# marksgraham/ddpm-ood

Hardware: AMD Instinct MI355X
Metric: reconstructions/sec (whole node), FashionMNIST 32x32 (higher is better)
Workload: dtype f32 (split-f16 MFMA products, fp32 accumulate)

## Files before the change

### ddpm_ood_amd/_lib.py

```python

from __future__ import annotations

import ctypes as C
import os
from pathlib import Path

import torch

_LIB = None
LIB_NAME = "libddpm_ood_hip.so"
ABI_VERSION = 10


class HipLibraryMissing(RuntimeError):
    pass


class ConvDesc(C.Structure):
    _fields_ = [
        ("in1", C.c_void_p), ("in2", C.c_void_p), ("C1", C.c_int), ("C2", C.c_int),
        ("w_packed", C.c_void_p), ("w_raw", C.c_void_p), ("bias", C.c_void_p),
        ("gscale", C.c_void_p), ("gshift", C.c_void_p),
        ("chan_add", C.c_void_p), ("chan_add_stride", C.c_int),
        ("residual", C.c_void_p), ("out", C.c_void_p),
        ("B", C.c_int), ("Cout", C.c_int),
        ("Hi", C.c_int), ("Wi", C.c_int), ("Ho", C.c_int), ("Wo", C.c_int),
        ("ksize", C.c_int), ("mode", C.c_int), ("act", C.c_int), ("force_direct", C.c_int),
        ("Di", C.c_int), ("Do", C.c_int), ("dims", C.c_int), ("depth_taps", C.c_int),
        ("w_folded", C.c_void_p), ("out_act", C.c_int), ("reserved", C.c_int), ("w_wino", C.c_void_p),
        ("scratch", C.c_void_p), ("scratch_floats", C.c_size_t), ("w_wino44", C.c_void_p),
        ("w_wino44h", C.c_void_p), ("stats_out", C.c_void_p), ("w_d3h", C.c_void_p),
    ]


MAX_LEVELS = 8


class UNetConfig(C.Structure):
    _fields_ = [
        ("spatial_dims", C.c_int), ("in_channels", C.c_int), ("out_channels", C.c_int),
        ("num_levels", C.c_int),
        ("num_channels", C.c_int * MAX_LEVELS), ("attention_levels", C.c_int * MAX_LEVELS),
        ("num_res_blocks", C.c_int * MAX_LEVELS), ("num_head_channels", C.c_int * MAX_LEVELS),
        ("norm_num_groups", C.c_int), ("norm_eps", C.c_float), ("use_proj_attn", C.c_int),
    ]


class GemmDesc(C.Structure):
    _fields_ = [
        ("A", C.c_void_p), ("B", C.c_void_p), ("C", C.c_void_p),
        ("M", C.c_int), ("N", C.c_int), ("K", C.c_int), ("k_inner", C.c_int),
        ("a_m", C.c_int64), ("a_k", C.c_int64), ("a_k_outer", C.c_int64),
        ("b_n", C.c_int64), ("b_k", C.c_int64), ("b_k_outer", C.c_int64),
        ("c_m", C.c_int64), ("c_n", C.c_int64),
        ("batch", C.c_int), ("batch_inner", C.c_int),
        ("a_batch", C.c_int64), ("a_batch_outer", C.c_int64), ("b_batch", C.c_int64), ("b_batch_outer", C.c_int64),
        ("c_batch", C.c_int64), ("c_batch_outer", C.c_int64),
        ("alpha", C.c_float), ("beta", C.c_float),
        ("scratch", C.c_void_p), ("scratch_floats", C.c_size_t),
        ("split_f16", C.c_int), ("reserved0", C.c_int),
    ]


SIGNATURES = {
    "ddpm_abi_version": (C.c_int, []),
    "ddpm_last_error": (C.c_char_p, []),
    "ddpm_conv_f32": (C.c_int, [C.POINTER(ConvDesc), C.c_void_p]),
    "ddpm_conv_scratch_floats": (C.c_size_t, [C.POINTER(ConvDesc)]),
    "ddpm_conv_takes_wino44h": (C.c_int, [C.POINTER(ConvDesc)]),
    "ddpm_conv_stats_parts": (C.c_int, [C.POINTER(ConvDesc)]),
    "ddpm_conv_kernel_name": (C.c_char_p, [C.POINTER(ConvDesc)]),
    "ddpm_conv_kernel_scratch_floats": (C.c_size_t, [C.POINTER(ConvDesc)]),
    "ddpm_conv_s2h_weight_halves": (C.c_size_t, [C.c_int, C.c_int]),
    "ddpm_pack_conv_s2h_weight": (C.c_int, [C.c_void_p, C.c_void_p, C.c_int, C.c_int, C.c_void_p]),
    "ddpm_conv_d3h_weight_halves": (C.c_size_t, [C.c_int, C.c_int]),
    "ddpm_pack_conv_d3h_weight": (C.c_int, [C.c_void_p, C.c_void_p, C.c_int, C.c_int, C.c_void_p]),
    "ddpm_conv_d1s_weight_halves": (C.c_size_t, [C.c_int, C.c_int]),
    "ddpm_pack_conv_d1s_weight": (C.c_int, [C.c_void_p, C.c_void_p, C.c_int, C.c_int, C.c_int, C.c_int, C.c_void_p]),
    "ddpm_conv1x1_h_weight_halves": (C.c_size_t, [C.c_int, C.c_int]),
    "ddpm_pack_conv1x1_h_weight": (C.c_int, [C.c_void_p, C.c_void_p, C.c_int, C.c_int, C.c_void_p]),
    "ddpm_packed_conv_weight_floats": (C.c_size_t, [C.c_int, C.c_int, C.c_int]),
    "ddpm_pack_conv_weight_f32": (C.c_int, [C.c_void_p, C.c_void_p, C.c_int, C.c_int, C.c_int, C.c_int, C.c_int,
                                            C.c_void_p]),
    "ddpm_pack_conv_weight_taps_f32": (C.c_int, [C.c_void_p, C.c_void_p, C.c_int, C.c_int, C.c_int, C.c_int, C.c_int,
                                                 C.c_void_p]),
    "ddpm_pack_conv3d_weight_f32": (C.c_int, [C.c_void_p, C.c_void_p, C.c_int, C.c_int, C.c_int, C.c_void_p]),
    "ddpm_packed_convtr_weight_floats": (C.c_size_t, [C.c_int, C.c_int, C.c_int]),
    "ddpm_pack_convtr_weight_f32": (C.c_int, [C.c_void_p, C.c_void_p, C.c_int, C.c_int, C.c_int, C.c_void_p]),
    "ddpm_conv3d_k4s2_cin1_f32": (C.c_int, [C.c_void_p] * 4 + [C.c_int] * 6 + [C.c_void_p]),
    "ddpm_convtr3d_parity_weights_f32": (C.c_int, [C.c_void_p, C.c_void_p, C.c_int, C.c_int, C.c_void_p]),
    "ddpm_parity_interleave3_f32": (C.c_int, [C.c_void_p, C.c_void_p, C.c_int64, C.c_int, C.c_int, C.c_int, C.c_void_p]),
    "ddpm_convtr3d_k4s2_cout1_f32": (C.c_int, [C.c_void_p] * 4 + [C.c_int] * 5 + [C.c_void_p]),
    "ddpm_wino_weight_floats": (C.c_size_t, [C.c_int, C.c_int]),
    "ddpm_pack_wino_weight_f32": (C.c_int, [C.c_void_p, C.c_void_p, C.c_int, C.c_int, C.c_void_p]),
    "ddpm_wino44_weight_floats": (C.c_size_t, [C.c_int, C.c_int]),
    "ddpm_pack_wino44_weight_f32": (C.c_int, [C.c_void_p, C.c_void_p, C.c_int, C.c_int, C.c_void_p]),
    "ddpm_pack_wino3d_weight_f32": (C.c_int, [C.c_void_p, C.c_void_p, C.c_int, C.c_int, C.c_void_p]),
    "ddpm_convnd_generic_f32": (C.c_int, [C.c_void_p] * 5 + [C.c_int] * 12 + [C.c_void_p]),
    "ddpm_wino44h_weight_halves": (C.c_size_t, [C.c_int, C.c_int]),
    "ddpm_pack_wino44h_weight": (C.c_int, [C.c_void_p, C.c_void_p, C.c_int, C.c_int, C.c_void_p]),
    "ddpm_pack_wino44h_weight3d": (C.c_int, [C.c_void_p, C.c_void_p, C.c_int, C.c_int, C.c_void_p]),
    "ddpm_pack_wino44_weight3d_f32": (C.c_int, [C.c_void_p, C.c_void_p, C.c_int, C.c_int, C.c_void_p]),
    "ddpm_folded_upsample_weight_floats": (C.c_size_t, [C.c_int, C.c_int]),
    "ddpm_fold_upsample_weight_f32": (C.c_int, [C.c_void_p, C.c_void_p, C.c_int, C.c_int, C.c_void_p]),
    "ddpm_gn_scale_shift_f32": (C.c_int, [C.c_void_p, C.c_void_p, C.c_int, C.c_int, C.c_void_p, C.c_void_p,
                                          C.c_void_p, C.c_void_p, C.c_int, C.c_int, C.c_int, C.c_float, C.c_void_p]),
    "ddpm_gn_finalize_f32": (C.c_int, [C.c_void_p, C.c_int, C.c_int, C.c_void_p, C.c_int, C.c_int, C.c_void_p, C.c_void_p,
                                       C.c_void_p, C.c_void_p, C.c_int, C.c_int, C.c_int, C.c_float, C.c_void_p]),
    "ddpm_channel_stats_f32": (C.c_int, [C.c_void_p, C.c_void_p, C.c_int, C.c_int, C.c_int, C.c_void_p]),
    "ddpm_attention_f32": (C.c_int, [C.c_void_p, C.c_void_p, C.c_void_p, C.c_int, C.c_int, C.c_int, C.c_int,
                                     C.c_float, C.c_void_p]),
    "ddpm_attention_scratch_floats": (C.c_size_t, [C.c_int, C.c_int, C.c_int, C.c_int]),
    "ddpm_attention_ws_f32": (C.c_int, [C.c_void_p, C.c_void_p, C.c_void_p, C.c_int, C.c_int, C.c_int, C.c_int,
                                        C.c_float, C.c_void_p, C.c_size_t, C.c_void_p]),
    "ddpm_timestep_embedding_f32": (C.c_int, [C.c_void_p, C.c_void_p, C.c_void_p, C.c_int, C.c_int, C.c_void_p]),
    "ddpm_add_noise_f32": (C.c_int, [C.c_void_p, C.c_void_p, C.POINTER(C.c_float), C.POINTER(C.c_float), C.c_float,
                                     C.c_void_p, C.c_int, C.c_int64, C.c_void_p]),
    "ddpm_plms_step_f32": (C.c_int, [C.c_void_p, C.c_void_p, C.c_void_p, C.c_void_p, C.c_void_p, C.c_int, C.c_int,
                                     C.c_float, C.c_float, C.c_float, C.c_float, C.c_float, C.c_void_p, C.c_int64,
                                     C.c_void_p]),
    "ddpm_ancestral_step_f32": (C.c_int, [C.c_void_p] * 4 + [C.c_int, C.c_int64, C.c_int, C.c_int] + [C.c_float] * 5
                                + [C.c_uint64, C.c_void_p, C.c_void_p]),
    "ddpm_randn_rows_f32": (C.c_int, [C.c_void_p, C.c_int, C.c_int64, C.c_uint64, C.c_void_p, C.c_void_p]),
    "ddpm_vlb_noise_rows_f32": (C.c_int, [C.c_void_p] * 5 + [C.c_int, C.c_void_p, C.c_int, C.c_int64, C.c_void_p]),
    "ddpm_vlb_term_rows_f32": (C.c_int, [C.c_void_p] * 6 + [C.c_int, C.c_int, C.c_int, C.c_float, C.c_void_p, C.c_void_p,
                                         C.c_int, C.c_int64, C.c_void_p]),
    "ddpm_clamp_mse_f32": (C.c_int, [C.c_void_p, C.c_void_p, C.c_float, C.c_void_p, C.c_int, C.c_int64, C.c_void_p]),
    "ddpm_vq_nearest_f32": (C.c_int, [C.c_void_p] * 5 + [C.c_int, C.c_int, C.c_int64, C.c_int, C.c_void_p]),
    "ddpm_vq_train_partials": (C.c_size_t, [C.c_int, C.c_int, C.c_int64]),
    "ddpm_vq_train_assign_f32": (C.c_int, [C.c_void_p] * 9 + [C.c_int, C.c_int, C.c_int64, C.c_int, C.c_float, C.c_void_p]),
    "ddpm_vq_train_update_f32": (C.c_int, [C.c_void_p] * 5 + [C.c_int, C.c_int, C.c_float, C.c_float, C.c_void_p]),
    "ddpm_vq_train_backward_f32": (C.c_int, [C.c_void_p] * 6 + [C.c_int, C.c_int, C.c_int64, C.c_float, C.c_void_p]),
    "ddpm_lpips_conv_f32": (C.c_int, [C.c_void_p] * 6 + [C.c_int] * 10 + [C.c_void_p]),
    "ddpm_maxpool3s2_f32": (C.c_int, [C.c_void_p, C.c_void_p, C.c_int64, C.c_int, C.c_int, C.c_void_p]),
    "ddpm_lpips_conv_biasmap_f32": (C.c_int, [C.c_void_p] * 4 + [C.c_int] * 9 + [C.c_void_p]),
    "ddpm_lpips_conv_mfma_supported": (C.c_int, [C.c_int] * 5),
    "ddpm_lpips_pack_conv_weight_f32": (C.c_int, [C.c_void_p, C.c_void_p, C.c_int, C.c_int, C.c_int, C.c_void_p]),
    "ddpm_lpips_conv_mfma_f32": (C.c_int, [C.c_void_p] * 4 + [C.c_int] * 7 + [C.c_void_p]),
    "ddpm_lpips_layer_f32": (C.c_int, [C.c_void_p] * 4 + [C.c_int] * 4 + [C.c_void_p]),
    "ddpm_sqerr_map_f32": (C.c_int, [C.c_void_p] * 3 + [C.c_int, C.c_int, C.c_int64, C.c_float, C.c_int, C.c_void_p]),
    "ddpm_lpips_layer_map_f32": (C.c_int, [C.c_void_p] * 4 + [C.c_int] * 3 + [C.c_int64, C.c_int64, C.c_void_p]),
    "ddpm_lpips_map_upsample_f32": (C.c_int, [C.c_void_p, C.c_void_p, C.c_int, C.c_int64] + [C.c_int] * 17
                                    + [C.c_float, C.c_int, C.c_void_p]),
    "ddpm_map_stats_update_f32": (C.c_int, [C.c_void_p, C.c_int, C.c_int64, C.c_int64, C.c_void_p, C.c_void_p, C.c_void_p]),
    "ddpm_map_zscore_f32": (C.c_int, [C.c_void_p] * 4 + [C.c_int, C.c_int, C.c_int64, C.c_float, C.c_void_p]),
    "ddpm_map_zscore_loo_f32": (C.c_int, [C.c_void_p] * 5 + [C.c_int, C.c_int, C.c_int64, C.c_int64, C.c_float, C.c_void_p]),
    "ddpm_map_blur_f32": (C.c_int, [C.c_void_p] * 3 + [C.c_int] * 4 + [C.c_void_p]),
    "ddpm_map_blur3d_f32": (C.c_int, [C.c_void_p] * 4 + [C.c_int] * 5 + [C.c_void_p]),
    "ddpm_lpips_map_upsample_view_f32": (C.c_int, [C.c_void_p, C.c_void_p, C.c_int, C.c_int64] + [C.c_int] * 15
                                         + [C.c_float, C.c_int, C.c_void_p]),
    "ddpm_map_mask_hist_f32": (C.c_int, [C.c_void_p, C.c_void_p, C.c_int, C.c_int64, C.c_float, C.c_float, C.c_int, C.c_int,
                                         C.c_void_p, C.c_void_p, C.c_int, C.c_void_p]),
    "ddpm_map_mask_counts_f32": (C.c_int, [C.c_void_p, C.c_void_p, C.c_int, C.c_int64, C.c_void_p, C.c_int, C.c_void_p, C.c_void_p]),
    "ddpm_map_label_u8": (C.c_int, [C.c_void_p, C.c_int, C.c_int, C.c_int, C.c_int, C.c_void_p, C.c_void_p, C.c_void_p]),
    "ddpm_map_label_f32": (C.c_int, [C.c_void_p, C.c_float, C.c_int, C.c_int, C.c_int, C.c_int, C.c_void_p, C.c_void_p, C.c_void_p]),
# ... 182 lines not shown
```

### ddpm_ood_amd/csrc/conv_wino44h.hip

```cpp
#include "wino44h_common.h"

namespace ddpm {

static int w44h_cus() {
  static int cus = 0;
  if (!cus) {
    int dev = 0;
    hipDeviceProp_t prop;
    if (hipGetDevice(&dev) == hipSuccess && hipGetDeviceProperties(&prop, dev) == hipSuccess)
      cus = prop.multiProcessorCount;
    if (cus <= 0) cus = 256;
  }
  return cus;
}

bool w44h_geom(const ddpm_conv_desc &d, W44HGeom &g, bool sizing) {
  const int Cin = d.C1 + d.C2;
  const bool is3d = d.dims == 3;
  const bool up = d.mode == DDPM_CONV_UPSAMPLE2;
  if (d.ksize != 3 || (!is3d && (d.Di > 1 || d.Do > 1)) || (d.mode != DDPM_CONV_NORMAL && !up)) return false;
  if (up) {
    if (!sw().up_wino44h || is3d || d.gscale || d.act != DDPM_ACT_NONE || d.C2 || d.chan_add || d.residual || d.out_act != DDPM_ACT_NONE)
      return false;
    if (d.Ho != 2 * d.Hi || d.Wo != 2 * d.Wi || d.Wo > 32) return false;
  }
  if ((d.out_act != DDPM_ACT_NONE && !(is3d && d.out_act == DDPM_ACT_RELU)) || d.act == DDPM_ACT_RELU) return false;
  if (d.gscale && d.act != DDPM_ACT_SILU) return false;
  if (is3d && (d.gscale || d.act != DDPM_ACT_NONE || d.C2 || d.chan_add)) return false;
  const int Dd = is3d ? (d.Di > 1 ? d.Di : 1) : 1;
  if (is3d && (d.Do > 1 ? d.Do : 1) != Dd) return false;
  if (Cin % 16 || (d.C2 > 0 && d.C1 % 4) || d.Cout % kK) return false;
  if ((d.Ho & 3) || (d.Wo & 3) || (!up && (d.Hi != d.Ho || d.Wi != d.Wo))) return false;
  if ((reinterpret_cast<uintptr_t>(d.out) | reinterpret_cast<uintptr_t>(d.residual)) & 15) return false;
  if ((double)d.B * (d.C1 > d.C2 ? d.C1 : d.C2) * Dd * d.Ho * d.Wo * 4 >= 2147483648.0) return false;
  if ((double)d.B * d.Cout * Dd * d.Ho * d.Wo * 4 >= 2147483648.0 * 2) return false;
  g.TWc = d.Wo / 4;
  g.THr = d.Ho / 4;
  const int per_img = g.TWc * g.THr;
  if (per_img >= kT) {
    if (kT % g.TWc) return false;
    g.TI = 1;
    g.TR = kT / g.TWc;
    if (g.THr % g.TR) return false;
    g.parts = g.THr / g.TR;
  } else {
    if (kT % per_img) return false;
    g.TI = kT / per_img;
    g.TR = g.THr;
    g.parts = 1;
  }
  if (is3d && g.TI != 1) return false;
  g.Cin = Cin;
  g.D = Dd;
  g.NIMG = d.B * Dd;
  g.NCHc = Cin / kC;
  g.kd0 = is3d && Dd == 1 ? 1 : 0;
  g.nkd = is3d && Dd > 1 ? 3 : 1;
  if (is3d && Dd > 1 && (d.depth_taps == 3 || d.depth_taps == 6)) {
    g.kd0 = d.depth_taps == 6 ? 1 : 0;
    g.nkd = 2;
  }
  g.nkd_w = is3d ? 3 : 1;
  g.NCH = g.nkd * g.NCHc;
  g.HW = d.Ho * d.Wo;
  g.up = up;
  g.HWin = up ? d.Hi * d.Wi : g.HW;
  g.CS = Dd * g.HW;
  g.prow = 4 * g.TR + 2;
  w44r_relayout(d, g);
  if (w44h_lds_bytes(g) > 160 * 1024) return false;
  if (64 % d.Wo) return false;
  const int rows = g.prow < d.Ho ? g.prow : d.Ho;
  g.UI = (rows * d.Wo + 63) / 64;
  g.NRT = g.TI * g.UI;
  if (g.TI == 1) {
    if (g.NRT != 9 && g.NRT != 10) return false;
    if ((rows - 1) * d.Wo < 64 * (g.NRT - 1)) return false;
  } else if (!((g.UI == 4 && rows * d.Wo == 256 && g.TI == 2) || (g.UI == 1 && rows * d.Wo == 64 && g.TI == 8))) {
    return false;
  }
  g.KT = d.Cout / kK;
  g.NIT = (g.NIMG + g.TI - 1) / g.TI;
  const long items = (long)g.KT * g.parts * g.NIT;
  const int cus = w44h_cus();
  const bool any_size = sw().conv_wino44 == 2;
  g.S = 1;
  g.pstride = 0;
  if (items < cus && !any_size) {
    if (is3d) return false;
    const int sp_max = sw().wino44_split;
    for (int sp = 4; sp >= 2; sp >>= 1)
      if (sp <= sp_max && items * sp <= cus && g.NCH % (2 * sp) == 0) { g.S = sp; break; }
    if (g.S == 1 || items * g.S * 4 < (long)cus * 3) return false;
    const size_t out_floats = (size_t)d.B * d.Cout * g.HW;
    if (!sizing && (!d.scratch || d.scratch_floats < g.S * out_floats)) return false;
    g.pstride = (long long)out_floats;
  }
  g.IPW = (int)((items + cus - 1) / cus);
  g.NS = g.parts * ((g.NIT + g.IPW - 1) / g.IPW) * g.S;
  while (g.S == 1 && items > cus && (long)g.KT * 8 <= cus && (long)g.KT * ((g.NS + 7) / 8) * 8 > cus && g.IPW < g.NIT) {
    ++g.IPW;
    g.NS = g.parts * ((g.NIT + g.IPW - 1) / g.IPW);
  }
  g.grid = g.KT * ((g.NS + 7) / 8) * 8;
  g.xitem = sw().w44h_xitem;
  g.rev = 0;
  g.xmap = (sw().wino44_xmap >= 0 ? sw().wino44_xmap != 0 : 0) && (8 % g.KT == 0);
  if (g.xmap) g.grid = 8 * ((g.NS + 8 / g.KT - 1) / (8 / g.KT));
  return true;
}

static bool w44h_enabled() {
  return sw().conv_wino44 != 0 && split_f16_on(sw().wino44_f16x3);
}

int conv_wino44h_stats_parts(const ddpm_conv_desc &d) {
  W44HGeom g;
  if (!w44h_enabled() || !d.w_wino44h || d.force_direct || d.dims == 3 || !w44h_geom(d, g, true)) return 0;
  const int per = g.TR * g.TWc;
  if (g.S != 1) return wino_split_reduce_stats_parts(g.HW);
  if ((per != 4 && per != 16 && per != 32) || g.parts > 8) return 0;
  return g.parts;
}

bool conv_wino44h_supported(const ddpm_conv_desc &d) {
  W44HGeom g;
  return w44h_enabled() && d.w_wino44h != nullptr && !d.force_direct && w44h_geom(d, g);
}

size_t conv_wino44h_scratch_floats(const ddpm_conv_desc &d) {
  W44HGeom g;
  if (!w44h_enabled() || !d.w_wino44h || d.force_direct || !w44h_geom(d, g, true) || g.S == 1) return 0;
  return (size_t)g.S * d.B * d.Cout * g.HW;
}

int launch_conv_wino44h(const ddpm_conv_desc &d, hipStream_t s) {
  W44HGeom g;
  if (!d.w_wino44h || !w44h_geom(d, g)) {
    set_error("conv_wino44h: unsupported shape");
    return DDPM_EINVAL;
  }
  ddpm_conv_desc dk = d;
  if (g.S > 1 || conv_wino44h_stats_parts(d) == 0) dk.stats_out = nullptr;
  if (g.S > 1) {
    dk.out = d.scratch;
    dk.bias = nullptr;
    dk.chan_add = nullptr;
    dk.residual = nullptr;
  }
  const double M = (double)g.NIMG * g.HW;
  const double flops = 2.0 * M * d.Cout * (double)g.Cin * 9 * g.nkd;
  const double bytes = 4.0 * ((g.up ? 0.25 : 1.0) * M * g.Cin + M * d.Cout * (d.residual ? 2 : 1) + (double)d.Cout * g.Cin * 9 * g.nkd);
  const char *kname = d.dims == 3 ? "conv3d_wino44h" : g.up ? "conv3x3_wino44h_up" : d.gscale ? "conv3x3_wino44h_gn_silu" : "conv3x3_wino44h";
  char kshape[160];
  if (g_prof_on && sw().prof_shapes) {
    snprintf(kshape, sizeof(kshape), "%s|%d+%d->%d@%dx%d", kname, d.C1, d.C2, d.Cout, d.Ho, d.Wo);
    kname = kshape;
  }
  ProfScope prof(s, kname, flops, bytes);
  static unsigned launch_parity = 0;
  g.rev = sw().w44r_serp ? (int)(launch_parity++ & 1) : 0;
  if (const int rc = launch_conv_wino44r(dk, g, w44h_lds_bytes(g), s)) return rc;
  if (g.S > 1) return launch_wino_split_reduce(d, g.S, g.pstride, g.HW, s);
  return 0;
}

__device__ __forceinline__ void wino44h_u(const float *w, double (&u)[6][6]) {
  const double G[6][3] = {{0.25, 0, 0},           {-1.0 / 6, -1.0 / 6, -1.0 / 6}, {-1.0 / 6, 1.0 / 6, -1.0 / 6},
                          {1.0 / 24, 1.0 / 12, 1.0 / 6}, {1.0 / 24, -1.0 / 12, 1.0 / 6},   {0, 0, 1}};
  double t[6][3];
  for (int r = 0; r < 6; ++r)
    for (int q = 0; q < 3; ++q) t[r][q] = G[r][0] * w[0 * 3 + q] + G[r][1] * w[1 * 3 + q] + G[r][2] * w[2 * 3 + q];
  for (int r = 0; r < 6; ++r)
    for (int c = 0; c < 6; ++c) u[r][c] = t[r][0] * G[c][0] + t[r][1] * G[c][1] + t[r][2] * G[c][2];
}

__global__ void wino44h_max_kernel(const float *__restrict__ src, unsigned *__restrict__ tail, int64_t total) {
  float m = 0.f;
  for (int64_t i = blockIdx.x * (int64_t)blockDim.x + threadIdx.x; i < total; i += (int64_t)gridDim.x * blockDim.x) {
    double u[6][6];
    wino44h_u(src + i * 9, u);
    for (int r = 0; r < 6; ++r)
      for (int c = 0; c < 6; ++c) m = fmaxf(m, fabsf((float)u[r][c]));
  }
  m = wave_max(m);
  if ((threadIdx.x & 63) == 0) atomicMax(tail, __float_as_uint(m));
}

__global__ void wino44h_pack_kernel(const float *__restrict__ src, uint16_t *__restrict__ dst, int Cout, int Cin, int nkd) {
  const int64_t total = (int64_t)Cout * Cin * nkd;
  const int nch = Cin / kC;
  float *tail = reinterpret_cast<float *>(dst + (size_t)kX * Cout * Cin * 2 * nkd);
  int e = 0;
  const float umax = tail[0];
  if (umax > 0.f) (void)frexpf(umax, &e);
  const int su = umax > 0.f ? 15 - e : 0;
  if (blockIdx.x == 0 && threadIdx.x == 0) tail[1] = ldexpf(1.f / kVScale, -su);
  const int trio_of[6] = {0, 1, 1, 2, 2, 0}, second_of[6] = {0, 0, 1, 0, 1, 1};
  for (int64_t i = blockIdx.x * (int64_t)blockDim.x + threadIdx.x; i < total; i += (int64_t)gridDim.x * blockDim.x) {
    const int kd = (int)(i % nkd);
    const int ci = (int)((i / nkd) % Cin), o = (int)(i / ((int64_t)nkd * Cin));
    double uu[6][6];
    wino44h_u(src + i * 9, uu);
    const int tile = o / kK, k64 = o % kK, ch = ci / kC, c8 = ci % kC;
    for (int r = 0; r < 6; ++r)
      for (int c = 0; c < 6; ++c) {
        const float u = ldexpf((float)uu[r][c], su);
        const _Float16 hi = (_Float16)u, lo = (_Float16)(u - (float)hi);
        const int s = second_of[r] * 6 + c;
        const size_t base = (((((size_t)tile * nkd + kd) * nch + ch) * 3 + trio_of[r]) * kPP + s) * 2;
        dst[((base + 0) * kK + k64) * kC + c8] = __builtin_bit_cast(uint16_t, hi);
        dst[((base + 1) * kK + k64) * kC + c8] = __builtin_bit_cast(uint16_t, lo);
      }
  }
}

size_t wino44h_weight_halves(int Cout, int Cin) {
  if (Cout % kK || Cin % 16) return 0;
  return (size_t)kX * Cout * Cin * 2 + kTail;
}

int launch_pack_wino44h_weight(const float *w_raw, uint16_t *w_wino44h, int Cout, int Cin, hipStream_t s, int nkd) {
  DDPM_CHECK_ARG(wino44h_weight_halves(Cout, Cin) != 0 && (nkd == 1 || nkd == 3), "wino44h pack: Cout %% 64 or Cin %% 16 != 0");
  const int64_t total = (int64_t)Cout * Cin * nkd;
  const int blocks = (int)((total + 255) / 256 > 4096 ? 4096 : (total + 255) / 256);
  unsigned *tail = reinterpret_cast<unsigned *>(w_wino44h + (size_t)kX * Cout * Cin * 2 * nkd);
  hipError_t e = hipMemsetAsync(tail, 0, kTail * sizeof(uint16_t), s);
  if (e != hipSuccess) {
    set_error("wino44h pack: %s", hipGetErrorString(e));
    return (int)e;
  }
  hipLaunchKernelGGL(wino44h_max_kernel, dim3(blocks), dim3(256), 0, s, w_raw, tail, total);
  DDPM_CHECK_LAUNCH();
  hipLaunchKernelGGL(wino44h_pack_kernel, dim3(blocks), dim3(256), 0, s, w_raw, w_wino44h, Cout, Cin, nkd);
  DDPM_CHECK_LAUNCH();
  return 0;
}

}
```

### ddpm_ood_amd/csrc/conv_wino44r.hip

```cpp
#include "wino44h_common.h"

namespace ddpm {

namespace {

constexpr int kVCB = 3 * kVSB;
static_assert(2 * kVCB == kRINGF * 4, "the V ring is the epilogue's four exchange slabs");

typedef int v4i_t __attribute__((ext_vector_type(4)));
typedef float v2f_t __attribute__((ext_vector_type(2)));

template <int O>
__device__ __forceinline__ void v_store_row_addtid(int m0base, const uint32_t (&hi6)[6], const uint32_t (&lo6)[6]) {
  asm volatile("s_mov_b32 m0, %0\n\ts_nop 1" ::"s"(m0base));
#pragma unroll
  for (int q = 0; q < 6; ++q) {
    asm volatile("ds_write_addtid_b32 %0 offset:%1" ::"v"(hi6[q]), "n"((2 * (O + q)) * (kT * 16)) : "memory");
    asm volatile("ds_write_addtid_b32 %0 offset:%1" ::"v"(lo6[q]), "n"((2 * (O + q) + 1) * (kT * 16)) : "memory");
  }
}

constexpr int w44r_up_job(int idx) {
  const int t = idx < 10 ? 0 : idx < 15 ? 1 : 2;
  const int k = idx - (t == 0 ? 0 : t == 1 ? 10 : 15);
  const int s = k < 2 ? k : k < 7 ? k + 1 : k + 2;
  const int row = t == 0 ? (s < 6 ? 0 : 5) : t == 1 ? 1 : (s < 6 ? 3 : 4);
  return (t * kVSB + 2 * s * (kT * 16)) | ((row * 6 + s % 6) << 16);
}
static_assert(kUSB == 2 * kVSB && 3 * kVSB < 65536, "w44r_up_job: U offset = 2 x V offset, below bit 16");

template <int T, int S>
__device__ __forceinline__ void v_store_pos_addtid(uint32_t hi, uint32_t lo) {
  asm volatile("ds_write_addtid_b32 %0 offset:%1" ::"v"(hi), "n"(T * kVSB + (2 * S) * (kT * 16)) : "memory");
  asm volatile("ds_write_addtid_b32 %0 offset:%1" ::"v"(lo), "n"(T * kVSB + (2 * S + 1) * (kT * 16)) : "memory");
}

template <class T>
__device__ __forceinline__ const T *uniform_ptr(const T *p) {
  const uint64_t v = reinterpret_cast<uint64_t>(p);
  const uint32_t lo = __builtin_amdgcn_readfirstlane((uint32_t)v), hi = __builtin_amdgcn_readfirstlane((uint32_t)(v >> 32));
  return reinterpret_cast<const T *>(((uint64_t)hi << 32) | lo);
}

}

template <bool AFFINE, int NRT, int UIT, bool RES, bool D3 = false, bool UP = false>
__global__ __launch_bounds__(512, 2) void conv_wino44r_kernel(const ddpm_conv_desc a, const W44HGeom g) {
  extern __shared__ __attribute__((aligned(16))) float smem[];
  constexpr bool ONEIMG = UIT == 0;
  constexpr int NGS = ONEIMG ? 1 : NRT / UIT;
  constexpr int GD = ONEIMG ? NRT : UIT;
  float *const P = smem + kRINGF;

  const int tid = threadIdx.x;
  const int lane = tid & 63, wave = __builtin_amdgcn_readfirstlane(tid >> 6);
  const int l31 = lane & 31, lhi = lane >> 5;
  const int cb = wave & 1, pg = wave >> 1;
  const bool lateprod = wave < 4;
  const bool silu = a.act == DDPM_ACT_SILU;

  const int xcd = blockIdx.x & 7, wj = blockIdx.x >> 3;
  int kt = wj % g.KT, slot = (wj / g.KT) * 8 + xcd;
  if (g.xmap) {
    kt = xcd % g.KT;
    slot = wj * (8 / g.KT) + xcd / g.KT;
  }
  if (slot >= g.NS) return;
  const int split = slot % g.S;
  slot /= g.S;
  const int part = slot % g.parts, it0 = (slot / g.parts) * g.IPW;
  const int nitems = min(g.IPW, g.NIT - it0);
  const int r0 = part * g.TR;
  const int n_first = it0 * g.TI, n_end = n_first + nitems * g.TI;
  const int istep = g.rev ? -g.TI : g.TI;
  const int NCHs = g.NCH / g.S, ch_lo = split * NCHs;
  float *const outp = a.out + (size_t)split * g.pstride;

  f32x16 acc8;
  reserve_agprs();

  const __amdgpu_buffer_rsrc_t rs_u = __builtin_amdgcn_make_buffer_rsrc(
      const_cast<uint16_t *>(a.w_wino44h), 0, (int)((size_t)kX * a.Cout * g.Cin * g.nkd_w * 4), 0x00020000);
  const int ukt = ((kt * g.nkd_w + g.kd0) * g.NCHc + ch_lo) * 3;
  int ua = (3 * pg * 2 + lhi) * (kK * 16) + (cb * 32 + l31) * 16;
  int va = 3 * pg * (2 * kT * 16) + l31 * 16;
  int upj[7] = {0, 0, 0, 0, 0, 0, 0};
  bool up7 = false;
  if constexpr (UP) {
#pragma unroll
    for (int j = 0; j < 7; ++j)
      upj[j] = __builtin_amdgcn_readfirstlane(pg == 0 ? w44r_up_job(j) : pg == 1 ? w44r_up_job(7 + j) : pg == 2 ? w44r_up_job(13 + j) : w44r_up_job(19 + (j < 6 ? j : 5)));
    up7 = pg == 0;
    ua = lhi * (kK * 16) + (cb * 32 + l31) * 16;
    va = l31 * 16;
  }

  auto barrier = [&]() __attribute__((always_inline)) {
    asm volatile("s_waitcnt lgkmcnt(0)\n\ts_barrier" ::: "memory");
    __builtin_amdgcn_sched_barrier(0);
  };
  auto zero_accumulators = [&]() __attribute__((always_inline)) {
    zero_pinned_tiles();
    if constexpr (UP) return;
    float z;
    asm volatile("v_mov_b32 %0, 0" : "=v"(z));
    acc8 = f32x16{z, z, z, z, z, z, z, z, z, z, z, z, z, z, z, z};
  };

#ifdef W44R_PROBE
  if (blockIdx.x == 0 && lane == 0 && a.scratch) reinterpret_cast<unsigned long long *>(a.scratch)[512 + wave * 32 + 31] = __builtin_readcyclecounter();
#endif
  auto zero_borders = [&]() __attribute__((always_inline)) {
    const v4f z4 = {0.f, 0.f, 0.f, 0.f};
    for (int i = tid; i < g.HS; i += 512) *reinterpret_cast<v4f *>(P + 4 * i) = z4;
    __syncthreads();
  };

  using I0 = std::integral_constant<int, 0>;
  using I1 = std::integral_constant<int, 1>;
  using I2 = std::integral_constant<int, 2>;

#ifdef W44R_PROBE
  int probe_cc = -100;
  int n_idx_probe = 0;
#define W44R_STAMP(i)                                                                                                  \
  if (blockIdx.x == 0 && probe_cc >= 4 && probe_cc < 8 && lane == 0 && a.scratch)                                      \
    reinterpret_cast<unsigned long long *>(a.scratch)[((wave * 4 + (probe_cc - 4)) * 16 + (i)) & 511] = __builtin_readcyclecounter();
#define W44R_FSTAMP(i)                                                                                                 \
  if (blockIdx.x == 0 && n_idx_probe == 0 && lane == 0 && a.scratch)                                                    \
    reinterpret_cast<unsigned long long *>(a.scratch)[512 + wave * 32 + (i)] = __builtin_readcyclecounter();
#else
#define W44R_STAMP(i)
#define W44R_FSTAMP(i)
#endif
  W44R_FSTAMP(0)
  const int ptask = (wave & 3) == 3 ? -1 : wave - (wave >> 2);
  const int pst = (ptask & 1) * 16 + (lane >> 2), pj = lane & 3;
  int tb0;
  {
    const int per = g.TR * g.TWc;
    const int ti = pst / per, rem = pst - ti * per;
    const int tr = rem / g.TWc, tc = rem - tr * g.TWc;
    tb0 = (pj >> 1) * g.HS + 2 * (pj & 1) * g.PCH + ti * g.IS + 4 * tr * g.PW + 4 * tc;
  }
  int vw0 = pst * 16 + 4 * pj;
  auto produce = [&](auto tc_, int cc) __attribute__((always_inline)) {
    constexpr int t = decltype(tc_)::value;
    constexpr bool t0 = t == 0;
    constexpr float c1 = t0 ? -5.f : t == 1 ? -2.f : -0.5f, c2 = t0 ? 4.f : c1, bm = t0 ? 0.f : t == 1 ? 1.f : 2.f;
    asm volatile("" : "+v"(tb0), "+v"(vw0));
    const int pb0 = tb0 + (cc & 1) * 2 * g.HS;
    float cA[2][6], cB[2][6];
#pragma unroll
    for (int c = 0; c < 2; ++c) {
// ... 657 lines not shown
```

### ddpm_ood_amd/csrc/wino44h_common.h

```cpp
#pragma once
#include <stdint.h>
#include <stdlib.h>

#include <type_traits>

#include "common.h"

namespace ddpm {

namespace {

typedef float f32x16 __attribute__((ext_vector_type(16)));
typedef float v4f __attribute__((ext_vector_type(4)));
typedef _Float16 h8 __attribute__((ext_vector_type(8)));
typedef _Float16 h2 __attribute__((ext_vector_type(2)));

constexpr int kT = 32;
constexpr int kK = 64;
constexpr int kC = 8;
constexpr int kX = 36;
constexpr int kPP = 12;
constexpr int kUSB = kPP * 2 * kK * 16;
constexpr int kVSB = kPP * 2 * kT * 16;
constexpr int kVB0 = 2 * kUSB;
// ... 58 lines not shown
  float v = 0.f;
  switch (r) {
#define X(n)                                                \
  case n:                                                   \
    asm volatile("v_accvgpr_read_b32 %0, a" #n : "=v"(v)); \
    break;
    W44H_REGS(X)
#undef X
  }
  return v;
}
__device__ __forceinline__ void mfma_v_pair_wait0(f32x16 &c, const h8 &a, const h8 &bh, const h8 &bl) {
  asm volatile("s_waitcnt lgkmcnt(0)\n\tv_mfma_f32_32x32x16_f16 %0, %1, %2, %0\n\tv_mfma_f32_32x32x16_f16 %0, %1, %3, %0\n\t"
               "s_nop 15\n\ts_nop 15\n\ts_nop 7"
               : "+v"(c) : "v"(a), "v"(bh), "v"(bl));
}
__device__ __forceinline__ h8 lds_b128(int byte_addr, int imm) {
  h8 v;
  asm volatile("ds_read_b128 %0, %1 offset:%2" : "=v"(v) : "v"(byte_addr), "n"(imm));
  return v;
}
__device__ __forceinline__ void sload2(const float *p, float &x0, float &x1) {
  asm volatile("s_load_dword %0, %2, 0x0\n\ts_load_dword %1, %2, 0x10\n\ts_waitcnt lgkmcnt(0)"
               : "=&s"(x0), "=&s"(x1) : "s"(p) : "memory");
}

__device__ __forceinline__ void sload8(const float *p, float (&x)[8]) {
  asm volatile("s_load_dword %0, %8, 0x0\n\ts_load_dword %1, %8, 0x10\n\ts_load_dword %2, %8, 0x20\n\ts_load_dword %3, %8, 0x30\n\t"
               "s_load_dword %4, %8, 0x40\n\ts_load_dword %5, %8, 0x50\n\ts_load_dword %6, %8, 0x60\n\ts_load_dword %7, %8, 0x70\n\t"
               "s_waitcnt lgkmcnt(0)"
               : "=&s"(x[0]), "=&s"(x[1]), "=&s"(x[2]), "=&s"(x[3]), "=&s"(x[4]), "=&s"(x[5]), "=&s"(x[6]), "=&s"(x[7])
               : "s"(p) : "memory");
}
__device__ __forceinline__ void sload8x2(const float *p, const float *r, float (&x)[8], float (&y)[8]) {
  asm volatile("s_load_dword %0, %16, 0x0\n\ts_load_dword %1, %16, 0x10\n\ts_load_dword %2, %16, 0x20\n\ts_load_dword %3, %16, 0x30\n\t"
               "s_load_dword %4, %16, 0x40\n\ts_load_dword %5, %16, 0x50\n\ts_load_dword %6, %16, 0x60\n\ts_load_dword %7, %16, 0x70\n\t"
               "s_load_dword %8, %17, 0x0\n\ts_load_dword %9, %17, 0x10\n\ts_load_dword %10, %17, 0x20\n\ts_load_dword %11, %17, 0x30\n\t"
               "s_load_dword %12, %17, 0x40\n\ts_load_dword %13, %17, 0x50\n\ts_load_dword %14, %17, 0x60\n\ts_load_dword %15, %17, 0x70\n\t"
               "s_waitcnt lgkmcnt(0)"
               : "=&s"(x[0]), "=&s"(x[1]), "=&s"(x[2]), "=&s"(x[3]), "=&s"(x[4]), "=&s"(x[5]), "=&s"(x[6]), "=&s"(x[7]),
                 "=&s"(y[0]), "=&s"(y[1]), "=&s"(y[2]), "=&s"(y[3]), "=&s"(y[4]), "=&s"(y[5]), "=&s"(y[6]), "=&s"(y[7])
               : "s"(p), "s"(r) : "memory");
}

__device__ __forceinline__ void bt6(const float (&w)[6], float (&t)[6]) {
  const float p = __builtin_fmaf(-4.f, w[2], w[4]), q = __builtin_fmaf(-4.f, w[1], w[3]);
  const float r = w[4] - w[2], s = w[3] - w[1];
  t[0] = __builtin_fmaf(4.f, w[0], __builtin_fmaf(-5.f, w[2], w[4]));
  t[1] = p + q;
  t[2] = p - q;
  t[3] = __builtin_fmaf(2.f, s, r);
  t[4] = __builtin_fmaf(-2.f, s, r);
  t[5] = __builtin_fmaf(4.f, w[1], __builtin_fmaf(-5.f, w[3], w[5]));
}
__device__ __forceinline__ void at4(float m0, float m1, float m2, float m3, float m4, float m5, float (&y)[4]) {
  const float s = m1 + m2, d = m1 - m2, u = m3 + m4, v = m3 - m4;
  y[0] = (m0 + s) + u;
  y[1] = __builtin_fmaf(2.f, v, d);
  y[2] = __builtin_fmaf(4.f, u, s);
  y[3] = __builtin_fmaf(8.f, v, d) + m5;
}

__device__ __forceinline__ void split_pair(float a, float b, uint32_t &hi, uint32_t &lo) {
  float la, lb;
  asm("v_cvt_pk_f16_f32 %0, %1, %2" : "=v"(hi) : "v"(a), "v"(b));
  asm("v_fma_mix_f32 %0, %1, -1.0, %2 op_sel:[0,0,0] op_sel_hi:[1,0,0]" : "=v"(la) : "v"(hi), "v"(a));
  asm("v_fma_mix_f32 %0, %1, -1.0, %2 op_sel:[1,0,0] op_sel_hi:[1,0,0]" : "=v"(lb) : "v"(hi), "v"(b));
  asm("v_cvt_pk_f16_f32 %0, %1, %2" : "=v"(lo) : "v"(la), "v"(lb));
}

}

struct W44HGeom {
  int TWc, THr;
  int TI, TR;
  int parts;
  int Cin, NCH, HW;
  int prow;
  int PW, IS, PCH;
  int HS;
  int UI;
  int NRT;
  int KT, NIT, IPW, NS, grid;
  int xmap;
  int xitem;
  int rev;
  int up, HWin;
  int S;
  long long pstride;
  int NIMG;
  int D;
  int CS;
  int NCHc;
  int kd0, nkd;
  int nkd_w;
};


bool w44h_geom(const ddpm_conv_desc &d, W44HGeom &g, bool sizing = false);
inline size_t w44h_lds_bytes(const W44HGeom &g) { return ((size_t)kRINGF + 4 * (size_t)g.HS) * sizeof(float); }
int launch_conv_wino44r(const ddpm_conv_desc &dk, const W44HGeom &g, size_t lds, hipStream_t s);
void w44r_relayout(const ddpm_conv_desc &d, W44HGeom &g);

}
```

### include/ddpm_ood_hip.h

```cpp
#ifndef DDPM_OOD_HIP_H
#define DDPM_OOD_HIP_H

#include <stddef.h>
#include <stdint.h>

#ifdef __cplusplus
extern "C" {
#endif

#define DDPM_ABI_VERSION 10

#define DDPM_EINVAL (-1)
#define DDPM_ENOPARAM (-2)
#define DDPM_EWORKSPACE (-3)

typedef void *ddpm_stream_t;

int ddpm_abi_version(void);
const char *ddpm_last_error(void);


#define DDPM_CONV_NORMAL 0
#define DDPM_CONV_STRIDE2 1
#define DDPM_CONV_UPSAMPLE2 2
#define DDPM_CONV_TRANSPOSE2 3
#define DDPM_ACT_NONE 0
#define DDPM_ACT_SILU 1
#define DDPM_ACT_RELU 2

typedef struct ddpm_conv_desc {
  const float *in1;
  const float *in2;
  int C1, C2;
  const float *w_packed;
  const float *w_raw;
  const float *bias;
  const float *gscale;
  const float *gshift;
  const float *chan_add;
  int chan_add_stride;
  const float *residual;
  float *out;
  int B, Cout;
  int Hi, Wi;
  int Ho, Wo;
  int ksize;
  int mode;
  int act;
  int force_direct;
  int Di, Do;
  int dims;
  int depth_taps;
  const float *w_folded;
  int out_act;
  int reserved;
  const float *w_wino;
  float *scratch;
  size_t scratch_floats;
  const float *w_wino44;
  const uint16_t *w_wino44h;
  float *stats_out;
  const uint16_t *w_d3h;
} ddpm_conv_desc;

int ddpm_conv_f32(const ddpm_conv_desc *d, ddpm_stream_t stream);
int ddpm_conv_takes_wino44h(const ddpm_conv_desc *desc);
size_t ddpm_conv_scratch_floats(const ddpm_conv_desc *d);
size_t ddpm_conv_d3h_weight_halves(int Cout, int Cin);
int ddpm_pack_conv_d3h_weight(const float *w_raw, uint16_t *dst, int Cout, int Cin, ddpm_stream_t stream);
size_t ddpm_conv_d1s_weight_halves(int Cout, int Cin);
int ddpm_pack_conv_d1s_weight(const float *w_raw, uint16_t *dst, int Cout, int Cin, int cout_offset, int Cout_total,
                              ddpm_stream_t stream);
size_t ddpm_conv1x1_h_weight_halves(int Cout, int Cin);
int ddpm_pack_conv1x1_h_weight(const float *w_raw, uint16_t *dst, int Cout, int Cin, ddpm_stream_t stream);
int ddpm_conv_stats_parts(const ddpm_conv_desc *d);
const char *ddpm_conv_kernel_name(const ddpm_conv_desc *desc);
size_t ddpm_conv_kernel_scratch_floats(const ddpm_conv_desc *desc);

size_t ddpm_packed_conv_weight_floats(int Cout, int Cin, int ksize);
int ddpm_pack_conv_weight_f32(const float *w_raw, float *w_packed, int Cout, int Cin, int ksize,
                              int cout_offset, int Cout_total, ddpm_stream_t stream);

int ddpm_pack_conv3d_weight_f32(const float *w_raw, float *w_packed, int Cout, int Cin, int ksize,
                                ddpm_stream_t stream);

size_t ddpm_packed_convtr_weight_floats(int Cout, int Cin, int dims);
int ddpm_pack_convtr_weight_f32(const float *w_raw, float *w_packed, int Cin, int Cout, int dims, ddpm_stream_t stream);

int ddpm_conv3d_k4s2_cin1_f32(const float *in, const float *w, const float *bias, float *out, int B, int Cout, int D,
                              int H, int W, int relu, ddpm_stream_t stream);
int ddpm_convnd_generic_f32(const float *in, const float *w, const float *bias, const float *residual, float *out, int B, int Cin,
                            int Cout, int Di, int Hi, int Wi, int dims, int ksize, int stride, int pad, int transposed, int relu,
                            ddpm_stream_t stream);
int ddpm_convtr3d_k4s2_cout1_f32(const float *in, const float *w, const float *bias, float *out, int B, int Cin, int D,
                                int H, int W, ddpm_stream_t stream);
int ddpm_convtr3d_parity_weights_f32(const float *w, float *g, int Cin, int Cout, ddpm_stream_t stream);
int ddpm_parity_interleave3_f32(const float *src, float *dst, int64_t planes, int D, int H, int W, ddpm_stream_t stream);

int ddpm_pack_conv_weight_taps_f32(const float *w_raw, float *w_packed, int Cout, int Cin, int ksize, int src_taps,
                                   int tap_off, ddpm_stream_t stream);

size_t ddpm_wino_weight_floats(int Cout, int Cin);
int ddpm_pack_wino_weight_f32(const float *w_raw, float *w_wino, int Cout, int Cin, ddpm_stream_t stream);

size_t ddpm_wino44_weight_floats(int Cout, int Cin);
int ddpm_pack_wino44_weight_f32(const float *w_raw, float *w_wino44, int Cout, int Cin, ddpm_stream_t stream);
size_t ddpm_wino44h_weight_halves(int Cout, int Cin);
int ddpm_pack_wino44h_weight(const float *w_raw, uint16_t *w_wino44h, int Cout, int Cin, ddpm_stream_t stream);
int ddpm_pack_wino44h_weight3d(const float *w_raw, uint16_t *w_wino44h, int Cout, int Cin, ddpm_stream_t stream);

size_t ddpm_conv_s2h_weight_halves(int Cout, int Cin);
int ddpm_pack_conv_s2h_weight(const float *w_raw, uint16_t *dst, int Cout, int Cin, ddpm_stream_t stream);

int ddpm_pack_wino3d_weight_f32(const float *w_raw, float *w_wino, int Cout, int Cin, ddpm_stream_t stream);
int ddpm_pack_wino44_weight3d_f32(const float *w_raw, float *w_wino44, int Cout, int Cin, ddpm_stream_t stream);

size_t ddpm_folded_upsample_weight_floats(int Cout, int Cin);
int ddpm_fold_upsample_weight_f32(const float *w_raw, float *w_folded, int Cout, int Cin, ddpm_stream_t stream);

int ddpm_gn_scale_shift_f32(const float *in1, const float *in2, int C1, int C2, const float *gamma,
                            const float *beta, float *scale, float *shift, int B, int HW, int groups,
                            float eps, ddpm_stream_t stream);

int ddpm_gn_finalize_f32(const float *st1, int parts1, int C1, const float *st2, int parts2, int C2, const float *gamma,
                         const float *beta, float *scale, float *shift, int B, int HW, int groups, float eps,
                         ddpm_stream_t stream);
int ddpm_channel_stats_f32(const float *in, float *stats, int B, int C, int HW, ddpm_stream_t stream);

int ddpm_attention_f32(const float *qkv, const float *residual, float *out, int B, int C, int N,
                       int num_heads, float scale, ddpm_stream_t stream);

int ddpm_timestep_embedding_f32(const int64_t *timesteps, const float *freqs, float *out, int B, int dim,
                                ddpm_stream_t stream);

int ddpm_add_noise_f32(const float *x0, const float *noise, const float *h_sqrt_ac, const float *h_sqrt_1m_ac,
                       float b_scale, float *out, int B, int64_t chw, ddpm_stream_t stream);

int ddpm_plms_step_f32(const float *sample, const float *e0, const float *e1, const float *e2, const float *e3,
                       int kind, int v_prediction, float v_a, float v_b, float sample_coeff, float coef_eps,
                       float denom, float *prev, int64_t numel, ddpm_stream_t stream);

#define DDPM_PREDICTION_EPSILON 0
#define DDPM_PREDICTION_V 1
#define DDPM_PREDICTION_SAMPLE 2
int ddpm_ancestral_step_f32(const float *sample, const float *model_output, float *prev, float *pred_original, int B,
                            int64_t row_numel, int prediction_type, int clip_sample, float sqrt_ac, float sqrt_1m_ac,
                            float c0, float ct, float sigma, uint64_t seed, const uint64_t *row_streams,
                            ddpm_stream_t stream);
int ddpm_randn_rows_f32(float *out, int B, int64_t row_numel, uint64_t seed, const uint64_t *row_streams,
                        ddpm_stream_t stream);

int ddpm_vlb_noise_rows_f32(const float *x0, const float *noise, const int32_t *row_src, const int32_t *row_t,
                            const float *coef, int T, float *x_t, int R, int64_t row_numel, ddpm_stream_t stream);
int ddpm_vlb_term_rows_f32(const float *x0, const float *x_t, const float *model_output, const int32_t *row_src,
                           const int32_t *row_t, const float *coef, int T, int prediction_type, int clip_sample,
                           float bin_width, float *term, float *kl_map, int R, int64_t row_numel, ddpm_stream_t stream);

int ddpm_clamp_mse_f32(const float *orig, float *recon, float b_scale, float *mse, int B, int64_t chw,
                       ddpm_stream_t stream);

// ... 234 lines not shown
```

Measured before the change: 1082.

## Choose Winograd block-to-XCD mapping by a modeled activation/weight traffic cost

Replaces the fixed block-to-work mapping of the wino44 conv kernel with a parameterised mapping (XK, XG, XR) that groups output-channel tiles and row parts across the 8 XCDs. A heuristic estimates the bytes moved for activations versus transformed weights under each grouping and picks the cheaper one, with the aim of improving per-XCD L2 reuse. A debug C entry point exposes the item map. The risk is that the cost model misjudges cache behaviour or that the grid rounding changes load balance.

Result: no change. 1089 (median of 6 runs) (+0.7%).

```diff
diff --git a/ddpm_ood_amd/_lib.py b/ddpm_ood_amd/_lib.py
--- a/ddpm_ood_amd/_lib.py
+++ b/ddpm_ood_amd/_lib.py
@@ -71,6 +71,7 @@
     "ddpm_conv_stats_parts": (C.c_int, [C.POINTER(ConvDesc)]),
     "ddpm_conv_kernel_name": (C.c_char_p, [C.POINTER(ConvDesc)]),
     "ddpm_conv_kernel_scratch_floats": (C.c_size_t, [C.POINTER(ConvDesc)]),
+    "ddpm_w44h_item_map": (C.c_int, [C.POINTER(ConvDesc), C.c_int, C.c_int, C.POINTER(C.c_int)]),
     "ddpm_conv_s2h_weight_halves": (C.c_size_t, [C.c_int, C.c_int]),
     "ddpm_pack_conv_s2h_weight": (C.c_int, [C.c_void_p, C.c_void_p, C.c_int, C.c_int, C.c_void_p]),
     "ddpm_conv_d3h_weight_halves": (C.c_size_t, [C.c_int, C.c_int]),
diff --git a/ddpm_ood_amd/csrc/conv_wino44h.hip b/ddpm_ood_amd/csrc/conv_wino44h.hip
--- a/ddpm_ood_amd/csrc/conv_wino44h.hip
+++ b/ddpm_ood_amd/csrc/conv_wino44h.hip
@@ -14,7 +14,31 @@
   return cus;
 }
 
-bool w44h_geom(const ddpm_conv_desc &d, W44HGeom &g, bool sizing) {
+static void w44h_set_map(W44HGeom &g, int code) {
+  const int xk = (code & 3) == 0 ? g.KT : (code & 3);
+  g.XK = (xk <= g.KT && g.KT % xk == 0 && 8 % (g.KT / xk) == 0) ? xk : g.KT;
+  g.XG = g.KT / g.XK;
+  g.XR = (code & 4) ? g.S * g.parts : 1;
+}
+static int w44h_map_code(const ddpm_conv_desc &d, const W44HGeom &g) {
+  if (g.S != 1 || d.dims == 3) return 0;
+  const double act = 4.0 * g.NIMG * g.Cin * g.HWin;
+  const double u = 144.0 * d.Cout * g.Cin * (g.up ? 25.0 / 36.0 : 1.0);
+  int best = 0;
+  double best_bytes = act + u * 8 * g.IPW;
+  for (int xk = 2; xk >= 1; --xk) {
+    if (xk >= g.KT || g.KT % xk || 8 % (g.KT / xk)) continue;
+    const int xg = g.KT / xk;
+    const double bytes = act * xg + u * 8 * g.IPW / xg;
+    if (bytes < best_bytes) best = xk, best_bytes = bytes;
+  }
+  return best | (g.parts > 1 ? 4 : 0);
+}
+static void w44h_pick_map(const ddpm_conv_desc &d, W44HGeom &g, int forced) {
+  w44h_set_map(g, forced >= 0 ? forced : sw().wino44_xmap >= 0 ? sw().wino44_xmap : w44h_map_code(d, g));
+}
+
+bool w44h_geom(const ddpm_conv_desc &d, W44HGeom &g, bool sizing, int map) {
   const int Cin = d.C1 + d.C2;
   const bool is3d = d.dims == 3;
   const bool up = d.mode == DDPM_CONV_UPSAMPLE2;
@@ -98,15 +122,14 @@
   }
   g.IPW = (int)((items + cus - 1) / cus);
   g.NS = g.parts * ((g.NIT + g.IPW - 1) / g.IPW) * g.S;
-  while (g.S == 1 && items > cus && (long)g.KT * 8 <= cus && (long)g.KT * ((g.NS + 7) / 8) * 8 > cus && g.IPW < g.NIT) {
+  w44h_pick_map(d, g, map);
+  while (g.S == 1 && items > cus && (long)g.KT * 8 <= cus && w44h_grid(g) > cus && g.IPW < g.NIT) {
     ++g.IPW;
     g.NS = g.parts * ((g.NIT + g.IPW - 1) / g.IPW);
   }
-  g.grid = g.KT * ((g.NS + 7) / 8) * 8;
+  g.grid = w44h_grid(g);
   g.xitem = sw().w44h_xitem;
   g.rev = 0;
-  g.xmap = (sw().wino44_xmap >= 0 ? sw().wino44_xmap != 0 : 0) && (8 % g.KT == 0);
-  if (g.xmap) g.grid = 8 * ((g.NS + 8 / g.KT - 1) / (8 / g.KT));
   return true;
 }
 
@@ -238,3 +261,15 @@
 }
 
 }
+
+using namespace ddpm;
+
+extern "C" int ddpm_w44h_item_map(const ddpm_conv_desc *d, int map, int block, int *out) {
+  W44HGeom g;
+  if (!d || !out || !w44h_geom(*d, g, true, map)) return 0;
+  if (block < 0 || block >= g.grid) return g.grid;
+  const W44HItems w = w44h_item_map(g, block);
+  const int v[12] = {w.kt, w.split, w.part, w.it0, w.nitems, g.KT, g.S, g.parts, g.NIT, g.TI, g.XK, g.XR};
+  for (int i = 0; i < 12; ++i) out[i] = v[i];
+  return g.grid;
+}
diff --git a/ddpm_ood_amd/csrc/conv_wino44r.hip b/ddpm_ood_amd/csrc/conv_wino44r.hip
--- a/ddpm_ood_amd/csrc/conv_wino44r.hip
+++ b/ddpm_ood_amd/csrc/conv_wino44r.hip
@@ -59,17 +59,9 @@
   const bool lateprod = wave < 4;
   const bool silu = a.act == DDPM_ACT_SILU;
 
-  const int xcd = blockIdx.x & 7, wj = blockIdx.x >> 3;
-  int kt = wj % g.KT, slot = (wj / g.KT) * 8 + xcd;
-  if (g.xmap) {
-    kt = xcd % g.KT;
-    slot = wj * (8 / g.KT) + xcd / g.KT;
-  }
-  if (slot >= g.NS) return;
-  const int split = slot % g.S;
-  slot /= g.S;
-  const int part = slot % g.parts, it0 = (slot / g.parts) * g.IPW;
-  const int nitems = min(g.IPW, g.NIT - it0);
+  const W44HItems wi = w44h_item_map(g, blockIdx.x);
+  if (wi.nitems == 0) return;
+  const int kt = wi.kt, split = wi.split, part = wi.part, it0 = wi.it0, nitems = wi.nitems;
   const int r0 = part * g.TR;
   const int n_first = it0 * g.TI, n_end = n_first + nitems * g.TI;
   const int istep = g.rev ? -g.TI : g.TI;
diff --git a/ddpm_ood_amd/csrc/wino44h_common.h b/ddpm_ood_amd/csrc/wino44h_common.h
--- a/ddpm_ood_amd/csrc/wino44h_common.h
+++ b/ddpm_ood_amd/csrc/wino44h_common.h
@@ -164,7 +164,7 @@
   int UI;
   int NRT;
   int KT, NIT, IPW, NS, grid;
-  int xmap;
+  int XK, XG, XR;
   int xitem;
   int rev;
   int up, HWin;
@@ -178,8 +178,31 @@
   int nkd_w;
 };
 
-
-bool w44h_geom(const ddpm_conv_desc &d, W44HGeom &g, bool sizing = false);
+struct W44HItems {
+  int kt, split, part, it0, nitems;
+};
+__host__ __device__ __forceinline__ W44HItems w44h_item_map(const W44HGeom &g, int block) {
+  const int xcd = block & 7, wj = block >> 3;
+  const int per = g.XK * g.XR;
+  const int q = wj % per;
+  W44HItems w;
+  w.kt = (xcd % g.XG) * g.XK + q % g.XK;
+  int slot = ((wj / per) * (8 / g.XG) + xcd / g.XG) * g.XR + q / g.XK;
+  w.split = slot % g.S;
+  slot /= g.S;
+  w.part = slot % g.parts;
+  w.it0 = (slot / g.parts) * g.IPW;
+  const int left = g.NIT - w.it0;
+  w.nitems = left <= 0 ? 0 : left < g.IPW ? left : g.IPW;
+  return w;
+}
+inline int w44h_grid(const W44HGeom &g) {
+  const int groups = g.NS / g.XR, per_round = 8 / g.XG;
+  return 8 * g.XK * g.XR * ((groups + per_round - 1) / per_round);
+}
+
+
+bool w44h_geom(const ddpm_conv_desc &d, W44HGeom &g, bool sizing = false, int map = -1);
 inline size_t w44h_lds_bytes(const W44HGeom &g) { return ((size_t)kRINGF + 4 * (size_t)g.HS) * sizeof(float); }
 int launch_conv_wino44r(const ddpm_conv_desc &dk, const W44HGeom &g, size_t lds, hipStream_t s);
 void w44r_relayout(const ddpm_conv_desc &d, W44HGeom &g);
diff --git a/include/ddpm_ood_hip.h b/include/ddpm_ood_hip.h
--- a/include/ddpm_ood_hip.h
+++ b/include/ddpm_ood_hip.h
@@ -76,6 +76,7 @@
 int ddpm_conv_stats_parts(const ddpm_conv_desc *d);
 const char *ddpm_conv_kernel_name(const ddpm_conv_desc *desc);
 size_t ddpm_conv_kernel_scratch_floats(const ddpm_conv_desc *desc);
+int ddpm_w44h_item_map(const ddpm_conv_desc *desc, int map, int block, int *out);
 
 size_t ddpm_packed_conv_weight_floats(int Cout, int Cin, int ksize);
 int ddpm_pack_conv_weight_f32(const float *w_raw, float *w_packed, int Cout, int Cin, int ksize,
```
